# 0beqz/realism-effects

Measured on NVIDIA H100. Metric: SSGI+denoise Mpixels/s at 4K, higher is better.
Workload: dtype f32 (fp16 accumulate planes)

## Files before the change

### realism_effects_b200/csrc/k_ssgi.cu

```cuda
#include "rfx_kernels.h"

#ifndef RFX_MARCH_BATCH
#define RFX_MARCH_BATCH 1
#endif
#ifndef RFX_K1_SIMPLE_MARCH
#define RFX_K1_SIMPLE_MARCH 0
#endif

namespace rfx {

#define SSGI_EPSILON 0.00001f
#define SSGI_ONE_MINUS_EPSILON (1.0f - 0.00001f)
#define PI_F 3.1415926535897932384626433832795f

RFX_D float lum_s(v3 a) { return dot(mk3(0.2125f, 0.7154f, 0.0721f), a); }
RFX_D float lg2a_(float x) { float r; asm("lg2.approx.ftz.f32 %0, %1;" : "=f"(r) : "f"(x)); return r; }

template <bool AP> RFX_D float rcp_(float x) { if (AP) { float r; asm("rcp.approx.ftz.f32 %0, %1;" : "=f"(r) : "f"(x)); return r; } return 1.0f / x; }
template <bool AP> RFX_D float div_(float a, float b) { return AP ? a * rcp_<true>(b) : a / b; }
template <bool AP> RFX_D float sqrt_(float x) { if (AP) { float r; asm("sqrt.approx.ftz.f32 %0, %1;" : "=f"(r) : "f"(x)); return r; } return sqrtf(x); }
template <bool AP> RFX_D v3 normalize_(v3 a) {
  if (AP) { float r; asm("rsqrt.approx.ftz.f32 %0, %1;" : "=f"(r) : "f"(dot(a, a))); return a * r; }
  return normalize(a);
}
// ... 210 lines not shown
    v3 pos[RFX_MARCH_BATCH];
    v2 uvs[RFX_MARCH_BATCH];
    float vzs[RFX_MARCH_BATCH];
    v3 p = hitPos;
#pragma unroll
    for (int k = 0; k < RFX_MARCH_BATCH; k++) {
      const int ii = min(i + k, a.steps - 1);
      const float cs = __ldg(cs_row + (ii - 1) * 256);
      p = p + dir * cs;
      pos[k] = p;
      uvs[k] = view_to_screen<SPARSE, AP>(a, p);
      vzs[k] = tex_r32f_nearest(a.viewz, uvs[k]);
    }
#pragma unroll
    for (int k = 0; k < RFX_MARCH_BATCH; k++) {
      if (!hit && i + k < a.steps) {
        const float diff = vzs[k] - pos[k].z;
        hitPos = pos[k];
        uv = uvs[k];
        if (diff >= 0.0f && diff < a.thickness) hit = true;
      }
    }
    i += RFX_MARCH_BATCH;
  }
#endif
  if (!hit) {
    hitPos = mk3(10.0e9f);
    return uv;
  }
  if (a.refine_steps == 0) return uv;
  dir = dir * 0.5f;
  hitPos = hitPos - dir;
  for (int r = 0; r < a.refine_steps; r++) {
    const v2 u = view_to_screen<SPARSE, AP>(a, hitPos);
    const float diff = tex_r32f_nearest(a.viewz, u) - hitPos.z;
    dir = dir * 0.5f;
    if (diff >= 0.0f) hitPos = hitPos - dir; else hitPos = hitPos + dir;
  }
  return view_to_screen<SPARSE, AP>(a, hitPos);
}

struct PixelMat {
  v3 diffuse;
  float roughness, metalness;
};

RFX_D float4 march_record(bool hit, v3 hitPos, v2 uv) { return hit ? make_float4(hitPos.x, hitPos.y, hitPos.z, 1.0f) : make_float4(10.0e9f, uv.x, uv.y, 0.0f); }

template <bool SPARSE, bool FAST, int PHASE>
RFX_D v3 doSample(const SsgiArgs& a, const PixelMat& m, v3 viewPos, v3 viewNormal, float roughnessSq, bool isDiffuseSample, bool isEnvSample,
                  float NoV, float NoL, float NoH, float LoH, int noiseB, v3& l, v3& hitPos, float& brdf, float& pdf, const float4* rec) {
  const float cosTheta = fmaxf(0.0f, dot(viewNormal, l));
  if (isDiffuseSample) {
    brdf = evalDisneyDiffuse<FAST>(NoL, NoV, LoH, roughnessSq, m.metalness);
    pdf = div_<FAST>(NoL, PI_F);
  } else {
    brdf = evalDisneySpecular<FAST>(roughnessSq, NoH, NoV, NoL);
    pdf = GGXVNDFPdf<FAST>(NoH, NoV, roughnessSq);
  }
  brdf *= cosTheta;
  pdf = fmaxf(SSGI_EPSILON, pdf);
  hitPos = viewPos;
  bool hit;
  v2 coords;
  if (PHASE == 2) {
    const float4 r = *rec;
    hit = r.w != 0.0f;
    l = l * (a.ray_distance / (float)a.steps);
    if (hit) {
      hitPos = mk3(r.x, r.y, r.z);
      coords = view_to_screen<SPARSE, FAST>(a, hitPos);
      if (a.refine_steps > 0) { l = l * 0.5f; for (int k = 0; k < a.refine_steps; k++) l = l * 0.5f; }
    } else {
      hitPos = mk3(10.0e9f);
      coords = mk2(r.y, r.z);
    }
  } else {
    coords = rayMarch<SPARSE, FAST>(a, l, hitPos, noiseB, hit);
  }
  const bool allowMissedRays = (a.flags & RFX_SSGI_MISSED_RAYS) != 0;
  if (!hit && !allowMissedRays) return getEnvColor<FAST>(a, l, roughnessSq, isDiffuseSample, isEnvSample);
  v2 vel = mk2(0.0f, 0.0f);
  if (a.velocity.p) { const float4 t = tex_f4_nearest(a.velocity, coords); vel = mk2(t.x, t.y); }
  const v2 ruv = coords - vel;
  const bool reproj_ok = ruv.x >= 0.0f && ruv.x <= 1.0f && ruv.y >= 0.0f && ruv.y <= 1.0f;
  const bool inner = FAST && reproj_ok && coords.x >= 0.15f && coords.x <= 1.0f - 0.15f && coords.y >= 0.15f && coords.y <= 1.0f - 0.15f;
  v3 envColor = mk3(0.0f);
  if (!inner) envColor = getEnvColor<FAST>(a, l, roughnessSq, isDiffuseSample, isEnvSample);
  v3 SSGI;
  if (reproj_ok) {
    v3 rgi = mk3(0.0f);
    if (a.accumulated.p) rgi = xyz(f4v(tex_f4_nearest(a.accumulated, ruv)));
    const float saturation = getSaturation<FAST>(m.diffuse);
    rgi = mix(rgi, mk3(lum_s(rgi)), (1.0f - roughnessSq) * saturation * 0.4f);
    const float border = 0.15f;
    float bf = smoothstep_<FAST>(0.0f, border, coords.x) * smoothstep_<FAST>(1.0f, 1.0f - border, coords.x) *
               smoothstep_<FAST>(0.0f, border, coords.y) * smoothstep_<FAST>(1.0f, 1.0f - border, coords.y);
    bf = sqrt_<FAST>(bf);
    SSGI = mix(envColor, rgi, bf);
  } else {
    return envColor;
  }
  if (allowMissedRays) {
    if (0.0f > lum_s(SSGI)) SSGI = mk3(0.0f);
  }
  return SSGI;
}

template <int MODE, bool IS, bool SPARSE, bool FAST, int PHASE>
#ifndef RFX_K1_MIN_BLOCKS
#define RFX_K1_MIN_BLOCKS 4
#endif
#ifndef RFX_K1_MARCH_MIN_BLOCKS
#define RFX_K1_MARCH_MIN_BLOCKS 8
#endif
__global__ void __launch_bounds__(kThreads, PHASE == 1 ? RFX_K1_MARCH_MIN_BLOCKS : RFX_K1_MIN_BLOCKS) ssgi_kernel(const __grid_constant__ SsgiArgs a) {
  int x, y;
  const bool in_rows = seg_pixel(a.segs, x, y);
  const bool active = x < a.W && y < a.H && in_rows;
  const uchar4 bn = __ldg(a.blue.tex + ((y + a.blue.shift.sy) % a.blue.size) * a.blue.size + ((x + a.blue.shift.sx) % a.blue.size));
  const v4 random = mk4((float)bn.x / 255.0f, (float)bn.y / 255.0f, (float)bn.z / 255.0f, (float)bn.w / 255.0f);

  v2 cdfUv = mk2(0.0f, 0.0f);
  float lambda = 0.0f;
  if (IS) {
    const float v = ld_r32f(a.env.marginal, nearest_i(random.x, a.env.marginal.w), 0);
    const float u = ld_r32f(a.env.conditional, nearest_i(random.y, a.env.conditional.w), nearest_i(v, a.env.conditional.h));
    cdfUv = mk2(u, v);
    const unsigned full = 0xffffffffu;
    const v2 ux = mk2(__shfl_xor_sync(full, u, 1), __shfl_xor_sync(full, v, 1));
    const v2 uy = mk2(__shfl_xor_sync(full, u, 2), __shfl_xor_sync(full, v, 2));
    const v2 sz = mk2(a.env.size_x, a.env.size_y);
    const v2 ddx = (ux - cdfUv) * sz, ddy = (uy - cdfUv) * sz;
    const float rho = fmaxf(length(ddx), length(ddy));
    lambda = rho > 0.0f ? (FAST ? lg2a_(rho) : log2f(rho)) : -1000.0f;
  }
  if (!active) return;

  const v2 vUv = pixel_uv(x, y, a.W, a.H);
  const float unpackedDepth = a.scaled ? tex_r32f_nearest(a.depth, vUv) : ld_r32f(a.depth, x, y);
  if (unpackedDepth == 1.0f) {
    if (PHASE == 1) return;
    v4 dl = mk4(0.0f, 0.0f, 0.0f, 1.0f);
    if (a.direct.p) dl = tex_h4_linear(a.direct, vUv);
    st_f4(a.out.p, a.out.pitch, x, y, packTwoVec4(dl, dl));
    return;
  }
  const float4 g = a.scaled ? tex_f4_nearest(a.gb, vUv) : ld_f4(a.gb, x, y);
  PixelMat m;
  m.diffuse = xyz(floatToVec4(g.x));
  const v3 worldNormal = unpackNormal(g.y);
  m.roughness = gb_roughness(g.z);
  m.metalness = gb_metalness(g.z);
  const float roughnessSq = clampf(m.roughness * m.roughness, 0.000001f, 1.0f);

  const float viewZ = ssgi_view_z(a, unpackedDepth);
  v3 viewPos;
  {
    const float clipW = a.cam.projection.m[2 * 4 + 3] * viewZ + a.cam.projection.m[3 * 4 + 3];
    v4 clip = mk4((vUv.x - 0.5f) * 2.0f, (vUv.y - 0.5f) * 2.0f, (viewZ - 0.5f) * 2.0f, 1.0f);
    clip = mk4(clip.x * clipW, clip.y * clipW, clip.z * clipW, clip.w * clipW);
    viewPos = xyz(mul(a.cam.projection_inverse, clip));
    viewPos.z = viewZ;
  }
  const v3 viewDir = normalize(viewPos);
  const v3 viewNormal = normalize(mul_dir_left(worldNormal, a.cam.camera_matrix_world));
  const v3 n = viewNormal;
  const v3 v = -viewDir;
  const float NoV = fmaxf(SSGI_EPSILON, dot(n, v));
  v3 V = mul_dir_left(v, a.cam.view_matrix);
  const v3 N = worldNormal;
  v3 T, B;
  Onb(N, T, B);
  V = ToLocal(T, B, N, V);
  const v3 f0 = mix(mk3(0.04f), m.diffuse, m.metalness);

  const float2 sc = __ldg(a.rot_table + bn.y);
  v3 Hh = SampleGGXVNDF_cs(V, roughnessSq, roughnessSq, random.x, sc.y, sc.x);
  if (Hh.z < 0.0f) Hh = -Hh;
  v3 l = normalize(reflect(-V, Hh));
  l = ToWorld(T, B, N, l);
  l = mul_dir_left(l, a.cam.camera_matrix_world);
  l = normalize(l);
  float NoL, NoH, LoH, VoH;
  calculateAngles<false>(l, v, n, NoL, NoH, LoH, VoH);

  bool isDiffuseSample = false;
  if (MODE == RFX_MODE_SSGI) {
    const v3 F = f0 + (mk3(1.0f) - f0) * pow5<FAST>(1.0f - VoH);
    float diffW = (1.0f - m.metalness) * lum_s(m.diffuse);
    float specW = lum_s(F);
    diffW = fmaxf(diffW, SSGI_EPSILON);
    specW = fmaxf(specW, SSGI_EPSILON);
    const float invW = 1.0f / (diffW + specW);
    diffW *= invW;
    isDiffuseSample = random.z < diffW;
  }

  float emsPdf = 1.0f, emsProbability = 0.0f;
  bool emsIsEnvSample = false;
  v3 envMisDir = mk3(0.0f);
  if (IS) {
    envMisDir = equirectUvToDirection<FAST>(cdfUv);
    const v3 color = env_trilinear(a.env, cdfUv, lambda);
    const float totalSum = a.env.total_sum_whole + a.env.total_sum_decimal;
    const float pdf0 = lum_s(color) / totalSum;
    emsPdf = a.env.size_x * a.env.size_y * pdf0;
    envMisDir = normalize(mul_dir_left(envMisDir, a.cam.camera_matrix_world));
    emsProbability = dot(envMisDir, viewNormal);
    emsProbability *= m.roughness;
    emsProbability = fminf(SSGI_ONE_MINUS_EPSILON, emsProbability);
    emsIsEnvSample = random.w < emsProbability;
    if (emsIsEnvSample) {
      emsPdf /= 1.0f - emsProbability;
      l = envMisDir;
      calculateAngles<FAST>(l, v, n, NoL, NoH, LoH, VoH);
    } else {
      emsPdf = 1.0f - emsProbability;
    }
  }
  const v3 diffuseRay = emsIsEnvSample ? envMisDir : cosineSampleHemisphere_cs<FAST>(viewNormal, random.x, sc.x, sc.y);
  const v3 specularRay = emsIsEnvSample ? envMisDir : l;

  float4* rec = PHASE != 0 ? (float4*)(a.rec + (long long)y * a.rec_pitch) + 2 * x : nullptr;
  if (PHASE == 1) {
    float4 r0 = make_float4(0.0f, 0.0f, 0.0f, 0.0f);
    if (MODE == RFX_MODE_SSGI && isDiffuseSample) {
      v3 d = diffuseRay, hp = viewPos;
      bool hit;
      const v2 uv = rayMarch<SPARSE, FAST>(a, d, hp, bn.z, hit);
      r0 = march_record(hit, hp, uv);
    }
    v3 d = specularRay, hp = viewPos;
    bool hit;
    const v2 uv = rayMarch<SPARSE, FAST>(a, d, hp, bn.z, hit);
    rec[0] = r0;
    rec[1] = march_record(hit, hp, uv);
    return;
  }
  v3 diffuseGI = mk3(0.0f), specularGI = mk3(0.0f), hitPos = mk3(0.0f);
  float brdf, pdf;
  bool haveDiffuse = false;
  if (MODE == RFX_MODE_SSGI && isDiffuseSample) {
    l = diffuseRay;
    calculateAngles<FAST>(l, v, n, NoL, NoH, LoH, VoH);
    v3 gi = doSample<SPARSE, FAST, PHASE>(a, m, viewPos, viewNormal, roughnessSq, true, emsIsEnvSample, NoV, NoL, NoH, LoH, bn.z, l, hitPos, brdf, pdf, rec);
    gi = gi * brdf;
    if (emsIsEnvSample) { const float aa = emsPdf * emsPdf, bb = pdf * pdf; gi = gi * div_<FAST>(aa, aa + bb); } else gi = vdiv_<FAST>(gi, pdf);
    gi = vdiv_<FAST>(gi, emsPdf);
    diffuseGI = mix(diffuseGI, gi, 1.0f / 1.0f);
    haveDiffuse = true;
  }
  l = specularRay;
  calculateAngles<FAST>(l, v, n, NoL, NoH, LoH, VoH);
  {
    v3 gi = doSample<SPARSE, FAST, PHASE>(a, m, viewPos, viewNormal, roughnessSq, isDiffuseSample, emsIsEnvSample, NoV, NoL, NoH, LoH, bn.z, l, hitPos, brdf, pdf,
                                          rec + 1);
    gi = gi * brdf;
    if (emsIsEnvSample) { const float aa = emsPdf * emsPdf, bb = pdf * pdf; gi = gi * div_<FAST>(aa, aa + bb); } else gi = vdiv_<FAST>(gi, pdf);
    gi = vdiv_<FAST>(gi, emsPdf);
    specularGI = mix(specularGI, gi, 1.0f / 1.0f);
  }
  const v3 specularHitPos = hitPos;
  if (a.flags & RFX_SSGI_USE_DIRECT_LIGHT) {
    v3 dl = mk3(0.0f);
    if (a.direct.p) dl = xyz(tex_h4_linear(a.direct, vUv));
    diffuseGI = diffuseGI + dl;
    specularGI = specularGI + dl;
  }
  float rayLength = 0.0f;
  if (!(hitPos.x > 10.0e8f)) {
    const v3 cameraPosWS = mk3(a.cam.camera_matrix_world.m[12], a.cam.camera_matrix_world.m[13], a.cam.camera_matrix_world.m[14]);
    const v3 hitPosWS = xyz(mul(a.cam.camera_matrix_world, mk4(specularHitPos, 1.0f)));
    const v3 dWS = cameraPosWS - hitPosWS;
    rayLength = sqrt_<FAST>(dot(dWS, dWS));
  }
  if (MODE == RFX_MODE_SSGI) {
    if (!haveDiffuse) diffuseGI = mk3(-1.0f);
    st_f4(a.out.p, a.out.pitch, x, y, packTwoVec4(mk4(diffuseGI, m.roughness), mk4(specularGI, rayLength)));
  } else {
    const float al = __uint_as_float(packHalf2x16(rayLength, m.roughness));
    st_f4(a.out.p, a.out.pitch, x, y, make_float4(specularGI.x, specularGI.y, specularGI.z, al));
  }
}

template <bool SPARSE>
RFX_D float tap_viewz(const SsgiArgs& a, v3 p) {
  f2 t;
  if (SPARSE) {
    const f2 c = f2fma(mkf2(p.x, p.y), mkf2(a.ps_x0, a.ps_y1), f2mul(mkf2(p.z), mkf2(a.ps_x2, a.ps_y2)));
    t = f2fma(c, mkf2(fx_rcp(-p.z)), mkf2(a.ps_hw, a.ps_hh));
  } else {
    const v2 uv = view_to_screen<false, true>(a, p);
    t = mkf2(uv.x * (float)a.W, uv.y * (float)a.H);
  }
  const int ix = clamp_idx(__float2int_rd(f2lo(t)), a.W - 1), iy = clamp_idx(__float2int_rd(f2hi(t)), a.H - 1);
  if (a.vz_tiled) return __ldg((const float*)a.viewz.p + (((iy >> 2) * a.vz_tiles_x + (ix >> 3)) * 32 + ((iy & 3) << 3) + (ix & 7)));
  return __ldg((const float*)a.viewz.p + (iy * a.vz_pitchw + ix));
}
RFX_D v3 fma3(v3 d, float s, v3 p) {
  const f2 xy = f2fma(mkf2(d.x, d.y), mkf2(s), mkf2(p.x, p.y));
  return mk3(f2lo(xy), f2hi(xy), fma_(d.z, s, p.z));
}
template <bool SPARSE, int BATCH>
RFX_D v2 march_fast(const SsgiArgs& a, v3& dir, v3& hitPos, int noiseB, bool& hit) {
  dir = dir * (a.ray_distance / (float)a.steps);
  hit = false;
  const float* cs_row = a.step_table + noiseB;
  v3 p = hitPos;
  for (int i = 1; i < a.steps && !hit; i += BATCH, cs_row += 256 * BATCH) {
    v3 q[BATCH];
    float z[BATCH];
    v3 t = p;
#pragma unroll
    for (int k = 0; k < BATCH; k++) {
      t = fma3(dir, __ldg(cs_row + 256 * k), t);
      q[k] = t;
      z[k] = tap_viewz<SPARSE>(a, t);
    }
#pragma unroll
    for (int k = 0; k < BATCH; k++) {
      if (!hit && i + k < a.steps) {
        p = q[k];
        const float d = z[k] - q[k].z;
        hit = d >= 0.0f && d < a.thickness;
      }
    }
  }
  if (!hit) {
    hitPos = mk3(10.0e9f);
    return view_to_screen<SPARSE, true>(a, p);
  }
  if (a.refine_steps > 0) {
    dir = dir * 0.5f;
    p = p - dir;
    for (int r = 0; r < a.refine_steps; r++) {
      const float diff = tap_viewz<SPARSE>(a, p) - p.z;
      dir = dir * 0.5f;
      p = diff >= 0.0f ? p - dir : p + dir;
    }
  }
  hitPos = p;
  return view_to_screen<SPARSE, true>(a, p);
}

template <bool SPARSE, bool PEER, int BATCH>
RFX_D v3 sample_fast(const SsgiArgs& a, v3 viewPos, v3 viewNormal, float roughnessSq, float metalness, float desat, bool isDiffuseSample, bool isEnvSample, float NoV,
                     float NoL, float NoH, float LoH, int noiseB, v3 l, v3& hitPos, float& brdf, float& pdf) {
  const float cosTheta = fmaxf(0.0f, dot(viewNormal, l));
  if (isDiffuseSample) {
    brdf = evalDisneyDiffuse<true>(NoL, NoV, LoH, roughnessSq, metalness);
    pdf = NoL * (1.0f / PI_F);
  } else {
    brdf = evalDisneySpecular<true>(roughnessSq, NoH, NoV, NoL);
    pdf = GGXVNDFPdf<true>(NoH, NoV, roughnessSq);
  }
  brdf *= cosTheta;
  pdf = fmaxf(SSGI_EPSILON, pdf);
  hitPos = viewPos;
  bool hit;
  const v2 coords = march_fast<SPARSE, BATCH>(a, l, hitPos, noiseB, hit);
  const bool allowMissedRays = (a.flags & RFX_SSGI_MISSED_RAYS) != 0;
  if (!hit && !allowMissedRays) return getEnvColor<true, true>(a, l, roughnessSq, isDiffuseSample, isEnvSample);
  v2 vel = mk2(0.0f, 0.0f);
  if (a.velocity.p) { const float4 t = tex_f4_nearest(a.velocity, coords); vel = mk2(t.x, t.y); }
  const v2 ruv = coords - vel;
  const bool reproj_ok = ruv.x >= 0.0f && ruv.x <= 1.0f && ruv.y >= 0.0f && ruv.y <= 1.0f;
  const bool inner = reproj_ok && coords.x >= 0.15f && coords.x <= 1.0f - 0.15f && coords.y >= 0.15f && coords.y <= 1.0f - 0.15f;
  v3 envColor = mk3(0.0f);
  if (!inner) envColor = getEnvColor<true, true>(a, l, roughnessSq, isDiffuseSample, isEnvSample);
  if (!reproj_ok) return envColor;
  v3 rgi = mk3(0.0f);
  if (a.accumulated.p) {
    const int ix = nearest_i(ruv.x, a.W), iy = nearest_i(ruv.y, a.H);
    const unsigned char* base = PEER ? peer_row_base(a.acc_peer, iy) : a.accumulated.p;
    const float4 t = __ldg((const float4*)(base + ((unsigned)iy * (unsigned)a.accumulated.pitch + (unsigned)ix * 16u)));
    rgi = mk3(t.x, t.y, t.z);
  }
  rgi = mix(rgi, mk3(lum_s(rgi)), desat);
  v3 SSGI = rgi;
  if (!inner) {
    const float border = 0.15f;
    float bf = smoothstep_<true>(0.0f, border, coords.x) * smoothstep_<true>(1.0f, 1.0f - border, coords.x) * smoothstep_<true>(0.0f, border, coords.y) *
               smoothstep_<true>(1.0f, 1.0f - border, coords.y);
    bf = sqrt_<true>(bf);
    SSGI = mix(envColor, rgi, bf);
  }
  if (allowMissedRays && 0.0f > lum_s(SSGI)) SSGI = mk3(0.0f);
  return SSGI;
}

template <int MODE, bool IS, bool SPARSE, bool PEER, int BATCH>
__global__ void __launch_bounds__(kThreads, RFX_K1_MIN_BLOCKS) ssgi_fast_kernel(const __grid_constant__ SsgiArgs a) {
  int x, y;
  const bool in_rows = seg_pixel(a.segs, x, y);
  const bool active = x < a.W && y < a.H && in_rows;
  const uchar4 bn = __ldg(a.blue.tex + blue_index(a.blue, x, y));
  const v4 random = mk4((float)bn.x / 255.0f, (float)bn.y / 255.0f, (float)bn.z / 255.0f, (float)bn.w / 255.0f);
  const unsigned full = 0xffffffffu;
  v2 cdfUv = mk2(0.0f, 0.0f);
  float lambda = 0.0f;
  if (IS) {
    const float v = ld_r32f(a.env.marginal, nearest_i(random.x, a.env.marginal.w), 0);
    const float u = ld_r32f(a.env.conditional, nearest_i(random.y, a.env.conditional.w), nearest_i(v, a.env.conditional.h));
    cdfUv = mk2(u, v);
    const v2 ux = mk2(__shfl_xor_sync(full, u, 1), __shfl_xor_sync(full, v, 1));
    const v2 uy = mk2(__shfl_xor_sync(full, u, 2), __shfl_xor_sync(full, v, 2));
    const v2 sz = mk2(a.env.size_x, a.env.size_y);
    const v2 ddx = (ux - cdfUv) * sz, ddy = (uy - cdfUv) * sz;
    const float rho = fmaxf(length(ddx), length(ddy));
    lambda = rho > 0.0f ? lg2a_(rho) : -1000.0f;
  }
  if (!active) return;
  const v2 vUv = pixel_uv(x, y, a.W, a.H);
  const float unpackedDepth = ld_r32f(a.depth, x, y);
  if (unpackedDepth == 1.0f) {
    v4 dl = mk4(0.0f, 0.0f, 0.0f, 1.0f);
    if (a.direct.p) dl = tex_h4_linear(a.direct, vUv);
    st_f4(a.out.p, a.out.pitch, x, y, packTwoVec4(dl, dl));
    return;
  }
  const float4 g = ld_f4(a.gb, x, y);
  PixelMat m;
  m.diffuse = xyz(floatToVec4(g.x));
  const v3 worldNormal = unpackNormal(g.y);
  m.roughness = gb_roughness(g.z);
  m.metalness = gb_metalness(g.z);
  const float roughnessSq = clampf(m.roughness * m.roughness, 0.000001f, 1.0f);
  const float viewZ = ssgi_view_z(a, unpackedDepth);
  v3 viewPos;
  {
    const float clipW = a.cam.projection.m[2 * 4 + 3] * viewZ + a.cam.projection.m[3 * 4 + 3];
    v4 clip = mk4((vUv.x - 0.5f) * 2.0f, (vUv.y - 0.5f) * 2.0f, (viewZ - 0.5f) * 2.0f, 1.0f);
    clip = mk4(clip.x * clipW, clip.y * clipW, clip.z * clipW, clip.w * clipW);
    viewPos = xyz(mul(a.cam.projection_inverse, clip));
    viewPos.z = viewZ;
  }
  const v3 viewDir = normalize(viewPos);
  const v3 viewNormal = normalize(mul_dir_left(worldNormal, a.cam.camera_matrix_world));
  const v3 n = viewNormal;
  const v3 v = -viewDir;
  const float NoV = fmaxf(SSGI_EPSILON, dot(n, v));
  v3 V = mul_dir_left(v, a.cam.view_matrix);
  const v3 N = worldNormal;
  v3 T, B;
  Onb(N, T, B);
  V = ToLocal(T, B, N, V);
  const v3 f0 = mix(mk3(0.04f), m.diffuse, m.metalness);
  const float2 sc = __ldg(a.rot_table + bn.y);
  v3 Hh = SampleGGXVNDF_cs(V, roughnessSq, roughnessSq, random.x, sc.y, sc.x);
  if (Hh.z < 0.0f) Hh = -Hh;
  v3 l = normalize(reflect(-V, Hh));
  l = ToWorld(T, B, N, l);
  l = mul_dir_left(l, a.cam.camera_matrix_world);
  l = normalize(l);
  float NoL, NoH, LoH, VoH;
  calculateAngles<false>(l, v, n, NoL, NoH, LoH, VoH);
  bool isDiffuseSample = false;
  if (MODE == RFX_MODE_SSGI) {
    const v3 F = f0 + (mk3(1.0f) - f0) * pow5<true>(1.0f - VoH);
    float diffW = (1.0f - m.metalness) * lum_s(m.diffuse);
    float specW = lum_s(F);
    diffW = fmaxf(diffW, SSGI_EPSILON);
    specW = fmaxf(specW, SSGI_EPSILON);
    const float invW = 1.0f / (diffW + specW);
    diffW *= invW;
    isDiffuseSample = random.z < diffW;
  }
  float emsPdf = 1.0f, emsProbability = 0.0f;
  bool emsIsEnvSample = false;
  v3 envMisDir = mk3(0.0f);
  if (IS) {
    envMisDir = equirectUvToDirection<true>(cdfUv);
    const v3 color = env_trilinear(a.env, cdfUv, lambda);
    const float totalSum = a.env.total_sum_whole + a.env.total_sum_decimal;
    const float pdf0 = lum_s(color) / totalSum;
    emsPdf = a.env.size_x * a.env.size_y * pdf0;
    envMisDir = normalize(mul_dir_left(envMisDir, a.cam.camera_matrix_world));
    emsProbability = dot(envMisDir, viewNormal);
    emsProbability *= m.roughness;
    emsProbability = fminf(SSGI_ONE_MINUS_EPSILON, emsProbability);
    emsIsEnvSample = random.w < emsProbability;
    if (emsIsEnvSample) {
      emsPdf /= 1.0f - emsProbability;
      l = envMisDir;
    } else {
      emsPdf = 1.0f - emsProbability;
    }
  }
  const float desat = (1.0f - roughnessSq) * getSaturation<true>(m.diffuse) * 0.4f;
  const float inv_ems = rcp_<true>(emsPdf);
  v3 diffuseGI = mk3(0.0f), specularGI, hitPos;
  float brdf, pdf;
  if (MODE == RFX_MODE_SSGI && isDiffuseSample) {
    const v3 dray = emsIsEnvSample ? envMisDir : cosineSampleHemisphere_cs<true>(viewNormal, random.x, sc.x, sc.y);
    calculateAngles<true>(dray, v, n, NoL, NoH, LoH, VoH);
    v3 gi = sample_fast<SPARSE, PEER, BATCH>(a, viewPos, viewNormal, roughnessSq, m.metalness, desat, true, emsIsEnvSample, NoV, NoL, NoH, LoH, bn.z, dray, hitPos, brdf, pdf);
    gi = gi * brdf;
    if (emsIsEnvSample) { const float aa = emsPdf * emsPdf, bb = pdf * pdf; gi = gi * div_<true>(aa, aa + bb); } else gi = vdiv_<true>(gi, pdf);
    diffuseGI = gi * inv_ems;
  }
  calculateAngles<true>(l, v, n, NoL, NoH, LoH, VoH);
  {
    v3 gi = sample_fast<SPARSE, PEER, BATCH>(a, viewPos, viewNormal, roughnessSq, m.metalness, desat, isDiffuseSample, emsIsEnvSample, NoV, NoL, NoH, LoH, bn.z, l, hitPos, brdf, pdf);
    gi = gi * brdf;
    if (emsIsEnvSample) { const float aa = emsPdf * emsPdf, bb = pdf * pdf; gi = gi * div_<true>(aa, aa + bb); } else gi = vdiv_<true>(gi, pdf);
    specularGI = gi * inv_ems;
  }
  float rayLength = 0.0f;
  if (!(hitPos.x > 10.0e8f)) {
    const v3 cameraPosWS = mk3(a.cam.camera_matrix_world.m[12], a.cam.camera_matrix_world.m[13], a.cam.camera_matrix_world.m[14]);
    const v3 hitPosWS = xyz(mul(a.cam.camera_matrix_world, mk4(hitPos, 1.0f)));
    const v3 dWS = cameraPosWS - hitPosWS;
    rayLength = sqrt_<true>(dot(dWS, dWS));
  }
  if (a.flags & RFX_SSGI_USE_DIRECT_LIGHT) {
    v3 dl = mk3(0.0f);
    if (a.direct.p) dl = xyz(tex_h4_linear(a.direct, vUv));
    diffuseGI = diffuseGI + dl;
    specularGI = specularGI + dl;
  }
  if (MODE == RFX_MODE_SSGI) {
    if (!isDiffuseSample) diffuseGI = mk3(-1.0f);
    st_f4(a.out.p, a.out.pitch, x, y, packTwoVec4(mk4(diffuseGI, m.roughness), mk4(specularGI, rayLength)));
  } else {
    const float al = __uint_as_float(packHalf2x16(rayLength, m.roughness));
    st_f4(a.out.p, a.out.pitch, x, y, make_float4(specularGI.x, specularGI.y, specularGI.z, al));
  }
}

template <int MODE, bool IS>
static void launch_ssgi_t(const SsgiArgs& a, dim3 grid, cudaStream_t s) {
#define RFX_K1_LAUNCH(SP, F, PH) ssgi_kernel<MODE, IS, SP, F, PH><<<grid, kThreads, 0, s>>>(a)
  if (a.phase == 0 && a.fast && !a.legacy_fast) {
    const bool peer = a.acc_peer.n > 1;
#define RFX_K1F(SP, PE, BA) ssgi_fast_kernel<MODE, IS, SP, PE, BA><<<grid, kThreads, 0, s>>>(a)
#define RFX_K1F_B(SP, PE) do { if (a.march_batch >= 4) RFX_K1F(SP, PE, 4); else if (a.march_batch <= 1) RFX_K1F(SP, PE, 1); else RFX_K1F(SP, PE, 2); } while (0)
    if (a.proj_sparse) { if (peer) RFX_K1F_B(true, true); else RFX_K1F_B(true, false); }
    else { if (peer) RFX_K1F_B(false, true); else RFX_K1F_B(false, false); }
#undef RFX_K1F_B
#undef RFX_K1F
  } else if (a.phase == 0) {
    if (a.proj_sparse) { if (a.fast) RFX_K1_LAUNCH(true, true, 0); else RFX_K1_LAUNCH(true, false, 0); }
    else { if (a.fast) RFX_K1_LAUNCH(false, true, 0); else RFX_K1_LAUNCH(false, false, 0); }
  } else if (a.phase == 1) {
    if (a.proj_sparse) RFX_K1_LAUNCH(true, true, 1); else RFX_K1_LAUNCH(false, true, 1);
  } else {
    if (a.proj_sparse) RFX_K1_LAUNCH(true, true, 2); else RFX_K1_LAUNCH(false, true, 2);
  }
#undef RFX_K1_LAUNCH
}

cudaError_t launch_ssgi(const SsgiArgs& a, cudaStream_t s) {
  dim3 grid((a.W + kTileW - 1) / kTileW, a.segs.tiles);
  const bool is = (a.flags & RFX_SSGI_IMPORTANCE_SAMPLING) != 0;
  if (a.mode == RFX_MODE_SSGI) {
    if (is) launch_ssgi_t<RFX_MODE_SSGI, true>(a, grid, s); else launch_ssgi_t<RFX_MODE_SSGI, false>(a, grid, s);
  } else {
    if (is) launch_ssgi_t<RFX_MODE_SSR, true>(a, grid, s); else launch_ssgi_t<RFX_MODE_SSR, false>(a, grid, s);
  }
  return cudaGetLastError();
}

}
```

### realism_effects_b200/csrc/rfx_api.cu

```cuda
#include <algorithm>
#include <cmath>
#include <cstdarg>
#include <cstdio>
#include <cstring>
#include <string>
#include <vector>

#include "rfx_kernels.h"

using namespace rfx;

struct rfx_ctx {
  int device = 0;
  cudaStream_t stream = nullptr;
  std::string err;
  uint64_t launches = 0;
  uchar4* blue = nullptr;
  int blue_size = 0;
  float2* rot_table = nullptr;
  float* step_table = nullptr;
  int step_table_steps = 0;
  bool env_set = false;
  double env_total = 0.0;
  EnvD env{};
  std::vector<void*> env_allocs;
  int fast_math = 1;
  void* nrd = nullptr;
  int nrd_w = 0, nrd_h = 0;
  size_t nrd_pitch = 0;
  bool nrd_reuse = false;
  void* viewz = nullptr;
  int viewz_w = 0, viewz_h = 0;
  size_t viewz_pitch = 0;
  bool viewz_reuse = false;
  int k1_phase = 0;
  void* k1rec = nullptr;
  size_t k1rec_pitch = 0;
  int k1rec_w = 0, k1rec_h = 0;
  const RowSegs* segs_override = nullptr;
  int k3_tma = 1;
  int k1_batch = 4;
  int compose_mode = 0;
  int debug_no_a_carry = 0;
  int k1_vz_tiled = 0;
  int legacy_k1 = 0;
  const PeerPV* peer_accumulated = nullptr;
};

static rfx_status fail(rfx_ctx* c, rfx_status st, const char* fmt, ...) {
  if (c) {
    char buf[512];
    va_list ap;
    va_start(ap, fmt);
    vsnprintf(buf, sizeof buf, fmt, ap);
    va_end(ap);
    c->err = buf;
  }
  return st;
}
#define CU(call)                                                                                        \
  do {                                                                                                  \
    cudaError_t e_ = (call);                                                                            \
    if (e_ != cudaSuccess) return fail(ctx, RFX_ERR_CUDA, "%s failed: %s", #call, cudaGetErrorString(e_)); \
  } while (0)

static const float kPi = 3.1415926535897932384626433832795f;

extern "C" {

int rfx_version(void) { return RFX_VERSION; }
uint32_t rfx_format_bytes(int32_t f) { return f == RFX_FMT_R32F ? 4u : f == RFX_FMT_RGBA32F ? 16u : f == RFX_FMT_RGBA16F ? 8u : f == RFX_FMT_RGBA8 ? 4u : 0u; }

rfx_status rfx_ctx_create(int device, rfx_ctx** out) {
  if (!out) return RFX_ERR_INVALID_ARG;
  *out = nullptr;
  int n = 0;
  if (cudaGetDeviceCount(&n) != cudaSuccess || device < 0 || device >= n) return RFX_ERR_CUDA;
  rfx_ctx* ctx = new rfx_ctx();
  ctx->device = device;
  if (const char* e = getenv("RFX_LEGACY_K1")) ctx->legacy_k1 = atoi(e);
  if (const char* e = getenv("RFX_K3_TMA")) ctx->k3_tma = atoi(e);
  if (const char* e = getenv("RFX_K1_BATCH")) ctx->k1_batch = atoi(e);
  if (const char* e = getenv("RFX_K1_VZ_TILED")) ctx->k1_vz_tiled = atoi(e);
  if (const char* e = getenv("RFX_DEBUG_NO_A_CARRY")) ctx->debug_no_a_carry = atoi(e);
  if (const char* e = getenv("RFX_COMPOSE_MODE")) ctx->compose_mode = atoi(e);
  if (cudaSetDevice(device) != cudaSuccess || cudaStreamCreateWithFlags(&ctx->stream, cudaStreamNonBlocking) != cudaSuccess) {
    delete ctx;
    return RFX_ERR_CUDA;
  }
  float2 rot[256];
  for (int k = 0; k < 256; k++) {
    volatile float r = (float)k / 255.0f;
    volatile float r2 = r * 2.0f;
    volatile float ang = r2 * kPi;
    rot[k].x = (float)std::sin((double)ang);
    rot[k].y = (float)std::cos((double)ang);
  }
  if (cudaMalloc(&ctx->rot_table, sizeof rot) != cudaSuccess || cudaMemcpy(ctx->rot_table, rot, sizeof rot, cudaMemcpyHostToDevice) != cudaSuccess) {
    cudaStreamDestroy(ctx->stream);
    delete ctx;
    return RFX_ERR_CUDA;
  }
  *out = ctx;
  return RFX_OK;
}

static void free_env(rfx_ctx* ctx) {
  for (void* p : ctx->env_allocs) cudaFree(p);
  ctx->env_allocs.clear();
  ctx->env_set = false;
  ctx->env = EnvD{};
}

void rfx_ctx_destroy(rfx_ctx* ctx) {
  if (!ctx) return;
  cudaSetDevice(ctx->device);
  cudaStreamSynchronize(ctx->stream);
  free_env(ctx);
  cudaFree(ctx->blue);
  cudaFree(ctx->rot_table);
  cudaFree(ctx->step_table);
  cudaFree(ctx->nrd);
  cudaFree(ctx->viewz);
  cudaFree(ctx->k1rec);
  cudaStreamDestroy(ctx->stream);
  delete ctx;
}
rfx_status rfx_ctx_set_fast_math(rfx_ctx* ctx, int32_t enable) {
  if (!ctx) return RFX_ERR_INVALID_ARG;
  ctx->fast_math = enable ? 1 : 0;
  return RFX_OK;
}
const char* rfx_last_error(const rfx_ctx* ctx) { return ctx ? ctx->err.c_str() : "null context"; }
void* rfx_ctx_stream(rfx_ctx* ctx) { return ctx ? (void*)ctx->stream : nullptr; }
rfx_status rfx_ctx_sync(rfx_ctx* ctx) {
  if (!ctx) return RFX_ERR_INVALID_ARG;
  CU(cudaStreamSynchronize(ctx->stream));
  return RFX_OK;
}
uint64_t rfx_launch_count(const rfx_ctx* ctx) { return ctx ? ctx->launches : 0; }

rfx_status rfx_blue_noise_set(rfx_ctx* ctx, const uint8_t* rgba8, uint32_t w, uint32_t h) {
  if (!ctx || !rgba8 || w != h || w == 0) return fail(ctx, RFX_ERR_INVALID_ARG, "blue noise must be a square RGBA8 image");
  CU(cudaSetDevice(ctx->device));
  cudaFree(ctx->blue);
  ctx->blue = nullptr;
  CU(cudaMalloc(&ctx->blue, (size_t)w * h * 4));
  CU(cudaMemcpy(ctx->blue, rgba8, (size_t)w * h * 4, cudaMemcpyHostToDevice));
  ctx->blue_size = (int)w;
  return RFX_OK;
}

rfx_status rfx_plane_alloc(rfx_ctx* ctx, int32_t format, uint32_t w, uint32_t h, rfx_plane* out) {
  if (!ctx || !out || w == 0 || h == 0 || rfx_format_bytes(format) == 0) return fail(ctx, RFX_ERR_INVALID_ARG, "plane_alloc: bad arguments");
  CU(cudaSetDevice(ctx->device));
  size_t pitch = ((size_t)w * rfx_format_bytes(format) + 255) & ~(size_t)255;
  void* p = nullptr;
  CU(cudaMalloc(&p, pitch * h));
  CU(cudaMemsetAsync(p, 0, pitch * h, ctx->stream));
  CU(cudaStreamSynchronize(ctx->stream));
  out->ptr = p; out->width = w; out->height = h; out->pitch = pitch; out->format = format; out->_reserved = 0;
  return RFX_OK;
}
rfx_status rfx_plane_free(rfx_ctx* ctx, rfx_plane* p) {
  if (!ctx || !p) return RFX_ERR_INVALID_ARG;
  CU(cudaSetDevice(ctx->device));
  CU(cudaFree(p->ptr));
  p->ptr = nullptr;
  return RFX_OK;
}
static cudaStream_t pick(rfx_ctx* ctx, void* s) { return s ? (cudaStream_t)s : ctx->stream; }
rfx_status rfx_plane_clear(rfx_ctx* ctx, void* stream, const rfx_plane* p) {
  if (!ctx || !p || !p->ptr) return RFX_ERR_INVALID_ARG;
  CU(cudaMemsetAsync(p->ptr, 0, p->pitch * p->height, pick(ctx, stream)));
  return RFX_OK;
}
rfx_status rfx_plane_upload(rfx_ctx* ctx, void* stream, const rfx_plane* dst, const void* host, uint64_t host_pitch) {
  if (!ctx || !dst || !dst->ptr || !host) return RFX_ERR_INVALID_ARG;
  size_t row = (size_t)dst->width * rfx_format_bytes(dst->format);
  if (host_pitch == 0) host_pitch = row;
  if (host_pitch == row && dst->pitch == row) CU(cudaMemcpyAsync(dst->ptr, host, row * dst->height, cudaMemcpyHostToDevice, pick(ctx, stream)));
  else CU(cudaMemcpy2DAsync(dst->ptr, dst->pitch, host, host_pitch, row, dst->height, cudaMemcpyHostToDevice, pick(ctx, stream)));
  return RFX_OK;
}
rfx_status rfx_plane_download(rfx_ctx* ctx, void* stream, const rfx_plane* src, void* host, uint64_t host_pitch) {
  if (!ctx || !src || !src->ptr || !host) return RFX_ERR_INVALID_ARG;
  size_t row = (size_t)src->width * rfx_format_bytes(src->format);
  if (host_pitch == 0) host_pitch = row;
  if (host_pitch == row && src->pitch == row) CU(cudaMemcpyAsync(host, src->ptr, row * src->height, cudaMemcpyDeviceToHost, pick(ctx, stream)));
  else CU(cudaMemcpy2DAsync(host, host_pitch, src->ptr, src->pitch, row, src->height, cudaMemcpyDeviceToHost, pick(ctx, stream)));
  return RFX_OK;
}
rfx_status rfx_plane_download_rows(rfx_ctx* ctx, void* stream, const rfx_plane* src, void* host, uint32_t row0, uint32_t row1) {
  if (!ctx || !src || !src->ptr || !host || row0 >= row1 || row1 > src->height) return RFX_ERR_INVALID_ARG;
  const size_t row = (size_t)src->width * rfx_format_bytes(src->format);
  const unsigned char* p = (const unsigned char*)src->ptr + (size_t)row0 * src->pitch;
  if (src->pitch == row) CU(cudaMemcpyAsync(host, p, row * (row1 - row0), cudaMemcpyDeviceToHost, pick(ctx, stream)));
  else CU(cudaMemcpy2DAsync(host, row, p, src->pitch, row, row1 - row0, cudaMemcpyDeviceToHost, pick(ctx, stream)));
  return RFX_OK;
}
rfx_status rfx_host_alloc(rfx_ctx* ctx, uint64_t bytes, void** out) {
  if (!ctx || !out) return RFX_ERR_INVALID_ARG;
  CU(cudaSetDevice(ctx->device));
  CU(cudaHostAlloc(out, bytes, cudaHostAllocDefault));
  return RFX_OK;
}
rfx_status rfx_host_free(rfx_ctx* ctx, void* p) {
  if (!ctx) return RFX_ERR_INVALID_ARG;
  CU(cudaFreeHost(p));
  return RFX_OK;
}

rfx_status rfx_env_clear(rfx_ctx* ctx) {
  if (!ctx) return RFX_ERR_INVALID_ARG;
  cudaSetDevice(ctx->device);
  cudaStreamSynchronize(ctx->stream);
  free_env(ctx);
  return RFX_OK;
}
rfx_status rfx_env_set(rfx_ctx* ctx, const rfx_env_desc* e) {
  if (!ctx || !e || !e->map_rgba16f || e->width == 0 || e->height == 0) return fail(ctx, RFX_ERR_INVALID_ARG, "env_set: bad arguments");
  CU(cudaSetDevice(ctx->device));
  CU(cudaStreamSynchronize(ctx->stream));
  free_env(ctx);
  int w = (int)e->width, h = (int)e->height, l = 0;
  EnvD d{};
  for (;;) {
    if (l >= 16) return fail(ctx, RFX_ERR_UNSUPPORTED, "env map too large");
    size_t pitch = ((size_t)w * 8 + 255) & ~(size_t)255;
    void* p = nullptr;
    CU(cudaMalloc(&p, pitch * h));
    ctx->env_allocs.push_back(p);
    d.mip[l] = PV{(const unsigned char*)p, w, h, (long long)pitch};
    if (l == 0) {
      CU(cudaMemcpy2DAsync(p, pitch, e->map_rgba16f, (size_t)w * 8, (size_t)w * 8, h, cudaMemcpyHostToDevice, ctx->stream));
    } else {
      cudaError_t ce = launch_env_downsample(d.mip[l - 1], OutV{(unsigned char*)p, (long long)pitch}, w, h, ctx->stream);
      if (ce != cudaSuccess) return fail(ctx, RFX_ERR_CUDA, "env downsample: %s", cudaGetErrorString(ce));
      ctx->launches++;
    }
    l++;
    if (w == 1 && h == 1) break;
    w = w > 1 ? w >> 1 : 1;
    h = h > 1 ? h >> 1 : 1;
  }
  d.levels = l;
  d.size_x = (float)e->width;
  d.size_y = (float)e->height;
  d.total_sum_whole = e->total_sum_whole;
  d.total_sum_decimal = e->total_sum_decimal;
  ctx->env_total = (double)e->total_sum_whole + (double)e->total_sum_decimal;
  if (e->marginal && e->conditional) {
    float *m = nullptr, *c = nullptr;
    CU(cudaMalloc(&m, (size_t)e->height * 4));
    ctx->env_allocs.push_back(m);
    CU(cudaMalloc(&c, (size_t)e->width * e->height * 4));
    ctx->env_allocs.push_back(c);
    CU(cudaMemcpyAsync(m, e->marginal, (size_t)e->height * 4, cudaMemcpyHostToDevice, ctx->stream));
    CU(cudaMemcpyAsync(c, e->conditional, (size_t)e->width * e->height * 4, cudaMemcpyHostToDevice, ctx->stream));
    d.marginal = PV{(const unsigned char*)m, (int)e->height, 1, (long long)e->height * 4};
    d.conditional = PV{(const unsigned char*)c, (int)e->width, (int)e->height, (long long)e->width * 4};
  }
  CU(cudaStreamSynchronize(ctx->stream));
  ctx->env = d;
  ctx->env_set = true;
  return RFX_OK;
}

rfx_status rfx_env_build(rfx_ctx* ctx, const void* map_rgba16f, uint32_t width, uint32_t height, int32_t flip_y) {
  if (!ctx || !map_rgba16f || width == 0 || height == 0) return fail(ctx, RFX_ERR_INVALID_ARG, "env_build: bad arguments");
  rfx_env_desc e{};
  e.map_rgba16f = map_rgba16f; e.width = width; e.height = height;
  rfx_status st = rfx_env_set(ctx, &e);
  if (st != RFX_OK) return st;
  const size_t n = (size_t)width * height;
  float *cdf_c = nullptr, *cdf_m = nullptr, *marg = nullptr, *cond = nullptr;
  double *row_sum = nullptr, *total = nullptr;
  CU(cudaMalloc(&cdf_c, n * 4)); CU(cudaMalloc(&cdf_m, (size_t)height * 4)); CU(cudaMalloc(&row_sum, (size_t)height * 8)); CU(cudaMalloc(&total, 8));
  CU(cudaMalloc(&marg, (size_t)height * 4)); ctx->env_allocs.push_back(marg);
  CU(cudaMalloc(&cond, n * 4)); ctx->env_allocs.push_back(cond);
  cudaError_t ce = launch_env_cdf(ctx->env.mip[0], flip_y ? 1 : 0, cdf_c, cdf_m, row_sum, total, marg, cond, ctx->stream);
  ctx->launches += 3;
  double t = 0.0;
  if (ce == cudaSuccess) ce = cudaMemcpyAsync(&t, total, 8, cudaMemcpyDeviceToHost, ctx->stream);
  if (ce == cudaSuccess) ce = cudaStreamSynchronize(ctx->stream);
  cudaFree(cdf_c); cudaFree(cdf_m); cudaFree(row_sum); cudaFree(total);
  if (ce != cudaSuccess) return fail(ctx, RFX_ERR_CUDA, "env_build: %s", cudaGetErrorString(ce));
  ctx->env.marginal = PV{(const unsigned char*)marg, (int)height, 1, (long long)height * 4};
  ctx->env.conditional = PV{(const unsigned char*)cond, (int)width, (int)height, (long long)width * 4};
  const double whole = (double)(int32_t)t;
  ctx->env.total_sum_whole = (float)whole;
  ctx->env.total_sum_decimal = (float)(t - whole);
  ctx->env_total = t;
  return RFX_OK;
}
rfx_status rfx_env_tables_download(rfx_ctx* ctx, float* marginal, float* conditional, double* total_sum) {
  if (!ctx) return RFX_ERR_INVALID_ARG;
  if (!ctx->env_set || !ctx->env.marginal.p) return fail(ctx, RFX_ERR_NOT_READY, "env_tables_download: no importance-sampling tables");
  CU(cudaStreamSynchronize(ctx->stream));
  if (marginal) CU(cudaMemcpy(marginal, ctx->env.marginal.p, (size_t)ctx->env.marginal.w * 4, cudaMemcpyDeviceToHost));
  if (conditional) CU(cudaMemcpy(conditional, ctx->env.conditional.p, (size_t)ctx->env.conditional.w * ctx->env.conditional.h * 4, cudaMemcpyDeviceToHost));
  if (total_sum) *total_sum = ctx->env_total;
  return RFX_OK;
}

}

static bool plane_ok(const rfx_plane* p, int fmt) {
  return p && p->ptr && p->format == fmt && p->pitch * (uint64_t)p->height < (1ull << 32) && (p->pitch % rfx_format_bytes(fmt)) == 0;
}
static bool pv(const rfx_plane* p, int fmt, PV& out) {
  if (!plane_ok(p, fmt)) return false;
  out = PV{(const unsigned char*)p->ptr, (int)p->width, (int)p->height, (long long)p->pitch};
  return true;
}
static bool ov(const rfx_plane* p, int fmt, OutV& out) {
  if (!plane_ok(p, fmt)) return false;
  out = OutV{(unsigned char*)p->ptr, (long long)p->pitch};
  return true;
}
static void cam_to_dev(const rfx_camera& c, CamD& d) {
  memcpy(d.projection.m, c.projection, 64);
  memcpy(d.projection_inverse.m, c.projection_inverse, 64);
  memcpy(d.camera_matrix_world.m, c.camera_matrix_world, 64);
  memcpy(d.view_matrix.m, c.view_matrix, 64);
  d.near_plane = c.near_plane;
  d.far_plane = c.far_plane;
  d.perspective = c.perspective;
}
static void pcg4d(uint32_t v[4]) {
  for (int i = 0; i < 4; i++) v[i] = v[i] * 1664525u + 1013904223u;
  v[0] += v[1] * v[3]; v[1] += v[2] * v[0]; v[2] += v[0] * v[1]; v[3] += v[1] * v[2];
  for (int i = 0; i < 4; i++) v[i] ^= v[i] >> 16;
  v[0] += v[1] * v[3]; v[1] += v[2] * v[0]; v[2] += v[0] * v[1]; v[3] += v[1] * v[2];
}
static rfx_status blue_for(rfx_ctx* ctx, int index, BlueD& b) {
  if (!ctx->blue) return fail(ctx, RFX_ERR_NOT_READY, "blue noise texture not set (rfx_blue_noise_set)");
  uint32_t ui = (uint32_t)index;
  uint32_t s1[4] = {ui, ui * 15843u, ui * 31u + 4566u, ui * 2345u + 58585u};
  pcg4d(s1);
  b.tex = ctx->blue;
  b.size = ctx->blue_size;
  b.shift.sx = (int)((s1[0] % 0x0fffffffu) % (uint32_t)ctx->blue_size);
  b.shift.sy = (int)((s1[1] % 0x0fffffffu) % (uint32_t)ctx->blue_size);
// ... 1025 lines not shown
```

Measured before the change: 1879.

## March diffuse and specular rays together in one interleaved loop

Replaces the two sequential per-ray march and shade calls with a joint two-ray march that issues depth taps for both rays per step, plus a two-ray shading pass that batches velocity and accumulation loads. The aim is more independent memory requests in flight per thread, hiding gather latency. The default march batch drops from 4 to 2 to offset the doubled per-iteration register use. Risks are higher register pressure and lower occupancy, and extra divergence when one ray finishes early.

Result: faster. 1937, median of 6 (+3.1%).

```diff
diff --git a/realism_effects_b200/csrc/k_ssgi.cu b/realism_effects_b200/csrc/k_ssgi.cu
--- a/realism_effects_b200/csrc/k_ssgi.cu
+++ b/realism_effects_b200/csrc/k_ssgi.cu
@@ -536,51 +536,8 @@
   const f2 xy = f2fma(mkf2(d.x, d.y), mkf2(s), mkf2(p.x, p.y));
   return mk3(f2lo(xy), f2hi(xy), fma_(d.z, s, p.z));
 }
-template <bool SPARSE, int BATCH>
-RFX_D v2 march_fast(const SsgiArgs& a, v3& dir, v3& hitPos, int noiseB, bool& hit) {
-  dir = dir * (a.ray_distance / (float)a.steps);
-  hit = false;
-  const float* cs_row = a.step_table + noiseB;
-  v3 p = hitPos;
-  for (int i = 1; i < a.steps && !hit; i += BATCH, cs_row += 256 * BATCH) {
-    v3 q[BATCH];
-    float z[BATCH];
-    v3 t = p;
-#pragma unroll
-    for (int k = 0; k < BATCH; k++) {
-      t = fma3(dir, __ldg(cs_row + 256 * k), t);
-      q[k] = t;
-      z[k] = tap_viewz<SPARSE>(a, t);
-    }
-#pragma unroll
-    for (int k = 0; k < BATCH; k++) {
-      if (!hit && i + k < a.steps) {
-        p = q[k];
-        const float d = z[k] - q[k].z;
-        hit = d >= 0.0f && d < a.thickness;
-      }
-    }
-  }
-  if (!hit) {
-    hitPos = mk3(10.0e9f);
-    return view_to_screen<SPARSE, true>(a, p);
-  }
-  if (a.refine_steps > 0) {
-    dir = dir * 0.5f;
-    p = p - dir;
-    for (int r = 0; r < a.refine_steps; r++) {
-      const float diff = tap_viewz<SPARSE>(a, p) - p.z;
-      dir = dir * 0.5f;
-      p = diff >= 0.0f ? p - dir : p + dir;
-    }
-  }
-  hitPos = p;
-  return view_to_screen<SPARSE, true>(a, p);
-}
-
-template <bool SPARSE, bool PEER, int BATCH>
-RFX_D v3 sample_fast(const SsgiArgs& a, v3 viewPos, v3 viewNormal, float roughnessSq, float metalness, float desat, bool isDiffuseSample, bool isEnvSample, float NoV,
-                     float NoL, float NoH, float LoH, int noiseB, v3 l, v3& hitPos, float& brdf, float& pdf) {
+RFX_D void sample_weights_fast(v3 viewNormal, float roughnessSq, float metalness, bool isDiffuseSample, float NoV, float NoL, float NoH, float LoH, v3 l,
+                               float& brdf, float& pdf) {
   const float cosTheta = fmaxf(0.0f, dot(viewNormal, l));
   if (isDiffuseSample) {
     brdf = evalDisneyDiffuse<true>(NoL, NoV, LoH, roughnessSq, metalness);
@@ -591,37 +548,132 @@
   }
   brdf *= cosTheta;
   pdf = fmaxf(SSGI_EPSILON, pdf);
-  hitPos = viewPos;
-  bool hit;
-  const v2 coords = march_fast<SPARSE, BATCH>(a, l, hitPos, noiseB, hit);
+}
+
+template <bool SPARSE, int BATCH>
+RFX_D void march2_fast(const SsgiArgs& a, v3 origin, int noiseB, bool active0, v3 (&dir)[2], bool (&hit)[2], v2 (&uv)[2], v3& hitPos1) {
+  const float scale = a.ray_distance / (float)a.steps;
+  v3 p[2];
+  bool run[2];
+#pragma unroll
+  for (int r = 0; r < 2; r++) {
+    dir[r] = dir[r] * scale;
+    p[r] = origin;
+    hit[r] = false;
+    run[r] = r == 1 || active0;
+  }
+  const float* cs_row = a.step_table + noiseB;
+  for (int i = 1; i < a.steps && (run[0] || run[1]); i += BATCH, cs_row += 256 * BATCH) {
+    float cs[BATCH];
+#pragma unroll
+    for (int k = 0; k < BATCH; k++) cs[k] = __ldg(cs_row + 256 * k);
+    v3 q[2][BATCH];
+    float z[2][BATCH];
+#pragma unroll
+    for (int r = 0; r < 2; r++) {
+      if (run[r]) {
+        v3 t = p[r];
+#pragma unroll
+        for (int k = 0; k < BATCH; k++) {
+          t = fma3(dir[r], cs[k], t);
+          q[r][k] = t;
+          z[r][k] = tap_viewz<SPARSE>(a, t);
+        }
+      }
+    }
+#pragma unroll
+    for (int r = 0; r < 2; r++) {
+      if (run[r]) {
+#pragma unroll
+        for (int k = 0; k < BATCH; k++) {
+          if (!hit[r] && i + k < a.steps) {
+            p[r] = q[r][k];
+            const float d = z[r][k] - q[r][k].z;
+            hit[r] = d >= 0.0f && d < a.thickness;
+          }
+        }
+        run[r] = !hit[r];
+      }
+    }
+  }
+  if (a.refine_steps > 0) {
+#pragma unroll
+    for (int r = 0; r < 2; r++) {
+      if (hit[r]) {
+        dir[r] = dir[r] * 0.5f;
+        p[r] = p[r] - dir[r];
+      }
+    }
+    for (int s = 0; s < a.refine_steps; s++) {
+      float z[2];
+#pragma unroll
+      for (int r = 0; r < 2; r++) if (hit[r]) z[r] = tap_viewz<SPARSE>(a, p[r]);
+#pragma unroll
+      for (int r = 0; r < 2; r++) {
+        if (hit[r]) {
+          const float diff = z[r] - p[r].z;
+          dir[r] = dir[r] * 0.5f;
+          p[r] = diff >= 0.0f ? p[r] - dir[r] : p[r] + dir[r];
+        }
+      }
+    }
+  }
+#pragma unroll
+  for (int r = 0; r < 2; r++) uv[r] = r == 1 || active0 ? view_to_screen<SPARSE, true>(a, p[r]) : mk2(0.0f, 0.0f);
+  hitPos1 = hit[1] ? p[1] : mk3(10.0e9f);
+}
+
+template <bool PEER>
+RFX_D void shade2_fast(const SsgiArgs& a, float roughnessSq, float desat, bool active0, const bool (&isDiffuseSample)[2], bool isEnvSample,
+                       const v3 (&l)[2], const bool (&hit)[2], const v2 (&coords)[2], v3 (&SSGI)[2]) {
   const bool allowMissedRays = (a.flags & RFX_SSGI_MISSED_RAYS) != 0;
-  if (!hit && !allowMissedRays) return getEnvColor<true, true>(a, l, roughnessSq, isDiffuseSample, isEnvSample);
-  v2 vel = mk2(0.0f, 0.0f);
-  if (a.velocity.p) { const float4 t = tex_f4_nearest(a.velocity, coords); vel = mk2(t.x, t.y); }
-  const v2 ruv = coords - vel;
-  const bool reproj_ok = ruv.x >= 0.0f && ruv.x <= 1.0f && ruv.y >= 0.0f && ruv.y <= 1.0f;
-  const bool inner = reproj_ok && coords.x >= 0.15f && coords.x <= 1.0f - 0.15f && coords.y >= 0.15f && coords.y <= 1.0f - 0.15f;
-  v3 envColor = mk3(0.0f);
-  if (!inner) envColor = getEnvColor<true, true>(a, l, roughnessSq, isDiffuseSample, isEnvSample);
-  if (!reproj_ok) return envColor;
-  v3 rgi = mk3(0.0f);
-  if (a.accumulated.p) {
-    const int ix = nearest_i(ruv.x, a.W), iy = nearest_i(ruv.y, a.H);
-    const unsigned char* base = PEER ? peer_row_base(a.acc_peer, iy) : a.accumulated.p;
-    const float4 t = __ldg((const float4*)(base + ((unsigned)iy * (unsigned)a.accumulated.pitch + (unsigned)ix * 16u)));
-    rgi = mk3(t.x, t.y, t.z);
-  }
-  rgi = mix(rgi, mk3(lum_s(rgi)), desat);
-  v3 SSGI = rgi;
-  if (!inner) {
-    const float border = 0.15f;
-    float bf = smoothstep_<true>(0.0f, border, coords.x) * smoothstep_<true>(1.0f, 1.0f - border, coords.x) * smoothstep_<true>(0.0f, border, coords.y) *
-               smoothstep_<true>(1.0f, 1.0f - border, coords.y);
-    bf = sqrt_<true>(bf);
-    SSGI = mix(envColor, rgi, bf);
-  }
-  if (allowMissedRays && 0.0f > lum_s(SSGI)) SSGI = mk3(0.0f);
-  return SSGI;
+  bool reproj[2], reproj_ok[2], inner[2];
+  v2 ruv[2];
+#pragma unroll
+  for (int r = 0; r < 2; r++) reproj[r] = (r == 1 || active0) && (hit[r] || allowMissedRays);
+  float4 vt[2];
+#pragma unroll
+  for (int r = 0; r < 2; r++) vt[r] = reproj[r] && a.velocity.p ? tex_f4_nearest(a.velocity, coords[r]) : make_float4(0.0f, 0.0f, 0.0f, 0.0f);
+#pragma unroll
+  for (int r = 0; r < 2; r++) {
+    ruv[r] = coords[r] - mk2(vt[r].x, vt[r].y);
+    reproj_ok[r] = reproj[r] && ruv[r].x >= 0.0f && ruv[r].x <= 1.0f && ruv[r].y >= 0.0f && ruv[r].y <= 1.0f;
+    inner[r] = reproj_ok[r] && coords[r].x >= 0.15f && coords[r].x <= 1.0f - 0.15f && coords[r].y >= 0.15f && coords[r].y <= 1.0f - 0.15f;
+  }
+  float4 ct[2];
+#pragma unroll
+  for (int r = 0; r < 2; r++) {
+    ct[r] = make_float4(0.0f, 0.0f, 0.0f, 0.0f);
+    if (reproj_ok[r] && a.accumulated.p) {
+      const int ix = nearest_i(ruv[r].x, a.W), iy = nearest_i(ruv[r].y, a.H);
+      const unsigned char* base = PEER ? peer_row_base(a.acc_peer, iy) : a.accumulated.p;
+      ct[r] = __ldg((const float4*)(base + ((unsigned)iy * (unsigned)a.accumulated.pitch + (unsigned)ix * 16u)));
+    }
+  }
+  v3 envColor[2];
+#pragma unroll
+  for (int r = 0; r < 2; r++) {
+    envColor[r] = mk3(0.0f);
+    if ((r == 1 || active0) && !inner[r]) envColor[r] = getEnvColor<true, true>(a, l[r], roughnessSq, isDiffuseSample[r], isEnvSample);
+  }
+#pragma unroll
+  for (int r = 0; r < 2; r++) {
+    if (!reproj_ok[r]) {
+      SSGI[r] = envColor[r];
+      continue;
+    }
+    v3 rgi = mk3(ct[r].x, ct[r].y, ct[r].z);
+    rgi = mix(rgi, mk3(lum_s(rgi)), desat);
+    SSGI[r] = rgi;
+    if (!inner[r]) {
+      const float border = 0.15f;
+      float bf = smoothstep_<true>(0.0f, border, coords[r].x) * smoothstep_<true>(1.0f, 1.0f - border, coords[r].x) *
+                 smoothstep_<true>(0.0f, border, coords[r].y) * smoothstep_<true>(1.0f, 1.0f - border, coords[r].y);
+      bf = sqrt_<true>(bf);
+      SSGI[r] = mix(envColor[r], rgi, bf);
+    }
+    if (allowMissedRays && 0.0f > lum_s(SSGI[r])) SSGI[r] = mk3(0.0f);
+  }
 }
 
 template <int MODE, bool IS, bool SPARSE, bool PEER, int BATCH>
@@ -724,22 +776,30 @@
   }
   const float desat = (1.0f - roughnessSq) * getSaturation<true>(m.diffuse) * 0.4f;
   const float inv_ems = rcp_<true>(emsPdf);
-  v3 diffuseGI = mk3(0.0f), specularGI, hitPos;
-  float brdf, pdf;
-  if (MODE == RFX_MODE_SSGI && isDiffuseSample) {
-    const v3 dray = emsIsEnvSample ? envMisDir : cosineSampleHemisphere_cs<true>(viewNormal, random.x, sc.x, sc.y);
-    calculateAngles<true>(dray, v, n, NoL, NoH, LoH, VoH);
-    v3 gi = sample_fast<SPARSE, PEER, BATCH>(a, viewPos, viewNormal, roughnessSq, m.metalness, desat, true, emsIsEnvSample, NoV, NoL, NoH, LoH, bn.z, dray, hitPos, brdf, pdf);
-    gi = gi * brdf;
-    if (emsIsEnvSample) { const float aa = emsPdf * emsPdf, bb = pdf * pdf; gi = gi * div_<true>(aa, aa + bb); } else gi = vdiv_<true>(gi, pdf);
-    diffuseGI = gi * inv_ems;
+  const bool diffuseRay = MODE == RFX_MODE_SSGI && isDiffuseSample;
+  const bool isDiffuse[2] = {true, isDiffuseSample};
+  v3 dir[2] = {l, l};
+  float brdf[2], pdf[2];
+  if (diffuseRay) {
+    dir[0] = emsIsEnvSample ? envMisDir : cosineSampleHemisphere_cs<true>(viewNormal, random.x, sc.x, sc.y);
+    calculateAngles<true>(dir[0], v, n, NoL, NoH, LoH, VoH);
+    sample_weights_fast(viewNormal, roughnessSq, m.metalness, true, NoV, NoL, NoH, LoH, dir[0], brdf[0], pdf[0]);
   }
   calculateAngles<true>(l, v, n, NoL, NoH, LoH, VoH);
-  {
-    v3 gi = sample_fast<SPARSE, PEER, BATCH>(a, viewPos, viewNormal, roughnessSq, m.metalness, desat, isDiffuseSample, emsIsEnvSample, NoV, NoL, NoH, LoH, bn.z, l, hitPos, brdf, pdf);
-    gi = gi * brdf;
-    if (emsIsEnvSample) { const float aa = emsPdf * emsPdf, bb = pdf * pdf; gi = gi * div_<true>(aa, aa + bb); } else gi = vdiv_<true>(gi, pdf);
-    specularGI = gi * inv_ems;
+  sample_weights_fast(viewNormal, roughnessSq, m.metalness, isDiffuseSample, NoV, NoL, NoH, LoH, l, brdf[1], pdf[1]);
+  bool hit[2];
+  v2 coords[2];
+  v3 hitPos;
+  march2_fast<SPARSE, BATCH>(a, viewPos, bn.z, diffuseRay, dir, hit, coords, hitPos);
+  v3 gis[2];
+  shade2_fast<PEER>(a, roughnessSq, desat, diffuseRay, isDiffuse, emsIsEnvSample, dir, hit, coords, gis);
+  v3 diffuseGI = mk3(0.0f), specularGI;
+#pragma unroll
+  for (int r = 0; r < 2; r++) {
+    if (r == 0 && !diffuseRay) continue;
+    v3 gi = gis[r] * brdf[r];
+    if (emsIsEnvSample) { const float aa = emsPdf * emsPdf, bb = pdf[r] * pdf[r]; gi = gi * div_<true>(aa, aa + bb); } else gi = vdiv_<true>(gi, pdf[r]);
+    if (r == 0) diffuseGI = gi * inv_ems; else specularGI = gi * inv_ems;
   }
   float rayLength = 0.0f;
   if (!(hitPos.x > 10.0e8f)) {
diff --git a/realism_effects_b200/csrc/rfx_api.cu b/realism_effects_b200/csrc/rfx_api.cu
--- a/realism_effects_b200/csrc/rfx_api.cu
+++ b/realism_effects_b200/csrc/rfx_api.cu
@@ -39,7 +39,7 @@
   int k1rec_w = 0, k1rec_h = 0;
   const RowSegs* segs_override = nullptr;
   int k3_tma = 1;
-  int k1_batch = 4;
+  int k1_batch = 2;
   int compose_mode = 0;
   int debug_no_a_carry = 0;
   int k1_vz_tiled = 0;
```
